# Shridhar2602/WebGPU-Path-Tracer

Measured on AMD Instinct MI355X. Metric: Mrays/s at 1080p, 8 bounces; achieved HBM GB/s vs roofline, higher is better.
Workload: dtype f32; 1 GPU; configs[1]: Cornell + monkey_968.obj (967 tris), 1920x1080, 64 spp, 8 bounces, stack_size 20; parallelism=1 GPU

## Files before the change

### webgpu-path-tracer_amd/csrc/ptmi.hip

```cpp
#include <dlfcn.h>
#include <hip/hip_runtime.h>
#include <rccl/rccl.h>

#include <algorithm>
#include <chrono>
#include <cmath>
#include <cstdio>
#include <cstdlib>
#include <condition_variable>
#include <cstring>
#include <functional>
#include <mutex>
#include <string>
#include <thread>
#include <vector>

#include "../../include/ptmi.h"
#include "ptmi_kernels.h"

using namespace ptmi;

int ptmi_bvhdev_build_scene(void* stream, const float* d_tris, uint32_t n, const int32_t* h_meshes, int n_meshes, const float* h_xforms, int n_xforms, float* d_rows,
                            float* d_tris_out, int* depth_out, uint32_t* bad_tri, int sah, uint32_t* n_nodes_out);
int ptmi_bvhdev_make_pairs(void* stream, const float* d_rows, uint32_t nn, float* d_pairs, int* d_leaf_table, uint32_t* n_multi);
// ... 49 lines not shown
  void loop() {
    std::unique_lock<std::mutex> lk(m);
    for (;;) {
      cv.wait(lk, [this] { return has_job || quit; });
      if (quit) return;
      std::function<int()> j = std::move(job);
      has_job = false;
      lk.unlock();
      const int r = j();
      lk.lock();
      result = r;
      done = true;
      cv.notify_all();
    }
  }
  void post(std::function<int()> j) {
    std::lock_guard<std::mutex> lk(m);
    if (!th.joinable()) th = std::thread([this] { loop(); });
    job = std::move(j);
    has_job = true;
    done = false;
    cv.notify_all();
  }
  int wait() {
    std::unique_lock<std::mutex> lk(m);
    cv.wait(lk, [this] { return done; });
    return result;
  }
  ~PeerWorker() {
    {
      std::lock_guard<std::mutex> lk(m);
      quit = true;
      cv.notify_all();
    }
    if (th.joinable()) th.join();
  }
};

struct Tuning {
  int lds_stack = 10;
  bool noabort = true;
  int waves_per_cu = 0;
  int bvh_teams = 16;
  int refill = kRefillThreshold, leaf_batch = kLeafBatch, bvh_range = (int)kBvhRange;
  int tail_waves_per_cu = 0;
  bool tail6 = true;
  int tail_park = 16;
  int bvh_carry = 32;
  int bvh_carry_slots = 1 << 18;
  int bvh_carry_last = 0;
  int bvh_carry_min_paths = 4 << 20, bvh_carry_min_depth = 12;
  int sort = -1;
  int shade_blocks_per_cu = 0;
  int tail_limit = -1;
  bool render_ahead = true;
  int path_budget_log2 = 30;
  int placement_tries = 6;
  bool debug_placement = false;
};

struct ptmi_ctx {
  int device = 0;
  hipStream_t stream = nullptr;
  std::string err;
  ptmi_params prm;
  Tuning tun;
  int num_cus = 256;

  std::vector<float> h_spheres, h_quads, h_xforms, h_mats, h_bvh;
  size_t n_tris_uploaded = 0;
  std::vector<int32_t> h_meshes;
  bool scene_dirty = true;

  DBuf d_quad_unit_n;
  DBuf d_bvh_rows;
  bool bvh_on_device = false;
  size_t bvh_dev_prims = 0;
  size_t bvh_dev_nodes = 0;
  bool bvh_dev_sah = false;
  bool bvh_dev_stale = false;
  int bvh_dev_depth = 0;
  DBuf d_spheres, d_sphere_info, d_quads, d_quad_mat, d_tris, d_pretri, d_trinorm, d_meshes, d_xforms, d_mats, d_pairs, d_leaf_table;
  DevScene S{};
  int bvh_depth = 0;
  bool has_unknown_material = false;
  int material_classes = 0;
  int shade_blocks_per_cu[16] = {0};

  int W = 0, H = 0;
  DBuf d_fb_own;
  float4* fb = nullptr;
  size_t fb_bytes = 0;
  int rank = 0, world = 1, tile = 64;

  size_t path_cap = 0;
  bool pixsum_alloc = false;
  size_t slot_cap = 0;
  DBuf d_q0[2], d_q1[2], d_q2[2], d_tp[2], d_hm[2];
  DBuf d_uv, d_acc, d_pixsum, d_touched, d_ctl, d_totals, d_scratch, d_spill, d_heads;
  DBuf d_carry[2];
  int ctl_cap = 0;

  struct Ahead {
    bool valid = false;
    float view[16];
    uint32_t frame0 = 0;
// ... 423 lines not shown
  const int a = step & 1, b = a ^ 1;
  P.in = Slots{c->d_q0[a].as<float4>(), c->d_q1[a].as<float4>(), c->d_q2[a].as<float4>()};
  P.out = Slots{c->d_q0[b].as<float4>(), c->d_q1[b].as<float4>(), c->d_q2[b].as<float4>()};
  P.hin = HitBuf{c->d_tp[a].as<float2>(), c->d_hm[a].as<uint32_t>()};
  P.hout = HitBuf{c->d_tp[b].as<float2>(), c->d_hm[b].as<uint32_t>()};
  P.uv = c->d_uv.as<float2>();
  P.acc = c->d_acc.as<float4>();
  P.pixsum = with_pixsum ? c->d_pixsum.as<float4>() : nullptr;
  P.touched = with_pixsum ? nullptr : c->d_touched.as<uint8_t>();
  P.cap = (uint32_t)c->slot_cap;
  return P;
}

const void* shade_kernel(bool is, bool so, bool cn, bool mu) {
  if (!is && !mu) {
    if (so) return cn ? reinterpret_cast<const void*>(&k_shade6<true, true>) : reinterpret_cast<const void*>(&k_shade6<true, false>);
    return cn ? reinterpret_cast<const void*>(&k_shade6<false, true>) : reinterpret_cast<const void*>(&k_shade6<false, false>);
  }
#define PTMI_SK(I, S, C, M) \
  if (is == I && so == S && cn == C && mu == M) return reinterpret_cast<const void*>(&k_shade<I, S, C, M>)
  PTMI_SK(false, false, false, true); PTMI_SK(false, false, true, true);
  PTMI_SK(false, true, false, true); PTMI_SK(false, true, true, true);
  PTMI_SK(true, false, false, false); PTMI_SK(true, false, false, true); PTMI_SK(true, false, true, false); PTMI_SK(true, false, true, true);
  PTMI_SK(true, true, false, false); PTMI_SK(true, true, false, true); PTMI_SK(true, true, true, false); PTMI_SK(true, true, true, true);
#undef PTMI_SK
  return nullptr;
}

int stack_alloc_for(const ptmi_ctx* c) { return std::max(1, std::min(c->prm.stack_size, std::max(c->bvh_depth, 1))); }

int env_int(const char* name, int dflt) {
  const char* v = getenv(name);
  return (v && *v) ? atoi(v) : dflt;
}
void load_tuning(ptmi_ctx* c) {
  Tuning t;
  t.lds_stack = std::max(1, env_int("PTMI_LDS_STACK", t.lds_stack));
  t.noabort = env_int("PTMI_NOABORT", 1) != 0;
  t.waves_per_cu = env_int("PTMI_WAVES_PER_CU", 0);
  t.bvh_teams = (int)std::max<uint32_t>(1, std::min<uint32_t>(kMaxTeams, (uint32_t)env_int("PTMI_BVH_TEAMS", t.bvh_teams)));
  t.refill = env_int("PTMI_REFILL", t.refill);
  t.leaf_batch = env_int("PTMI_LEAF_BATCH", t.leaf_batch);
  t.bvh_range = std::max(64, std::min(1 << 16, env_int("PTMI_BVH_RANGE", t.bvh_range))) & ~63;
  t.tail_waves_per_cu = std::max(0, std::min(32, env_int("PTMI_TAIL_WAVES_PER_CU", t.tail_waves_per_cu)));
  t.tail6 = env_int("PTMI_TAIL6", 1) != 0;
  t.tail_park = std::max(0, std::min(63, env_int("PTMI_TAIL_PARK", t.tail_park)));
  t.bvh_carry = std::max(0, env_int("PTMI_BVH_CARRY", t.bvh_carry));
  t.bvh_carry_slots = std::max(64, std::min(1 << 22, env_int("PTMI_BVH_CARRY_SLOTS", t.bvh_carry_slots)));
  t.bvh_carry_last = std::max(0, env_int("PTMI_BVH_CARRY_LAST", t.bvh_carry_last));
  t.bvh_carry_min_paths = std::max(0, env_int("PTMI_BVH_CARRY_MIN_PATHS", t.bvh_carry_min_paths));
  t.bvh_carry_min_depth = std::max(0, env_int("PTMI_BVH_CARRY_MIN_DEPTH", t.bvh_carry_min_depth));
  t.sort = env_int("PTMI_SORT", -1);
  t.shade_blocks_per_cu = env_int("PTMI_SHADE_BLOCKS_PER_CU", 0);
  t.tail_limit = env_int("PTMI_TAIL_LIMIT", -1);
  t.render_ahead = env_int("PTMI_RENDER_AHEAD", 1) != 0;
  t.path_budget_log2 = std::max(16, std::min(31, env_int("PTMI_PATH_BUDGET_LOG2", t.path_budget_log2)));
  t.placement_tries = env_int("PTMI_PLACEMENT_TRIES", t.placement_tries);
  t.debug_placement = getenv("PTMI_DEBUG_PLACEMENT") != nullptr;
  c->tun = t;
}

int launch_intersect(ptmi_ctx* c, const Paths& P, StepCtl* ctl, uint32_t max_items, bool with_prims, const RenderConst* first_rc = nullptr, const Carry& cy = Carry{}) {
  unsigned long long* tot = c->d_totals.as<unsigned long long>();
  const uint32_t pgrid = std::max<uint32_t>(1, std::min<uint32_t>((max_items + kBlock - 1) / kBlock, (uint32_t)c->num_cus * 32));
  if (with_prims) {
    ScopedSpan sp(c, T_PRIMS);
    if (c->counters) hipLaunchKernelGGL(k_prims<true>, dim3(pgrid), dim3(kBlock), 0, c->stream, c->S, P, ctl, c->d_heads.as<uint32_t>(), tot);
    else hipLaunchKernelGGL(k_prims<false>, dim3(pgrid), dim3(kBlock), 0, c->stream, c->S, P, ctl, c->d_heads.as<uint32_t>(), tot);
  }
  if (c->S.n_nodes <= 0) return PTMI_OK;
  ScopedSpan sp(c, T_BVH);
  const Tuning& tun = c->tun;
  const int sa = stack_alloc_for(c);
  const int le = std::min(sa, tun.lds_stack);
  const int se = sa - le;
  const size_t lds = (size_t)le * 2 * 64 * sizeof(int) + kCandSlots * sizeof(uint32_t);
  const bool noabort = c->bvh_depth < c->prm.stack_size && tun.noabort;
  int waves_per_cu = (int)std::min<size_t>(28, (size_t)(160 * 1024) / (lds + 64));
  if (tun.waves_per_cu > 0) waves_per_cu = tun.waves_per_cu;
  const uint32_t want = (max_items + 63) / 64;
  const uint32_t grid = std::max<uint32_t>(1, std::min<uint32_t>(want, (uint32_t)c->num_cus * (uint32_t)waves_per_cu));
  const uint32_t n_teams = (uint32_t)tun.bvh_teams;
  HIP_TRY(c, c->d_spill.ensure(std::max<size_t>(16, (size_t)std::max<uint32_t>(grid, (uint32_t)c->num_cus * 32) * (size_t)se * 64 * sizeof(int2))));
  const int thr = tun.refill, leaf_batch = tun.leaf_batch;
  const uint32_t range_cap = (uint32_t)tun.bvh_range;
  float4 cam = make_float4(0.0f, 0.0f, 0.0f, 0.0f);
  if (first_rc) cam = make_float4(first_rc->cam_o[0], first_rc->cam_o[1], first_rc->cam_o[2], 1.0f);
#define PTMI_LAUNCH_BVH(CNT, NA)                                                                                                                                       \
  hipLaunchKernelGGL((k_bvh2<CNT, NA>), dim3(grid), dim3(64), lds, c->stream, c->S, P, ctl, c->d_heads.as<uint32_t>(), n_teams, c->prm.stack_size, le, se, \
                     c->d_spill.as<int2>(), thr, leaf_batch, tot, range_cap, cam, cy)
  if (c->counters) {
    if (noabort) PTMI_LAUNCH_BVH(true, true);
    else PTMI_LAUNCH_BVH(true, false);
  } else {
    if (noabort) PTMI_LAUNCH_BVH(false, true);
    else PTMI_LAUNCH_BVH(false, false);
  }
#undef PTMI_LAUNCH_BVH
  HIP_TRY(c, hipGetLastError());
  return PTMI_OK;
}

int launch_tail(ptmi_ctx* c, const RenderConst& rc, const Paths& P, StepCtl* ctl, int first, uint32_t limit, const Carry& cy_in) {
  Carry cy = cy_in;
  cy.park_below = (c->S.n_nodes > 0 && c->bvh_depth >= 12) ? c->tun.tail_park : 0;
  const int sa = stack_alloc_for(c) + (cy.park_below > 0 ? 3 : 0);
// ... 130 lines not shown
    for (int k = 0; k < 10; k++) {
      if (ok && cand[k].p) {
        losers.bufs.emplace_back();
        std::swap(losers.bufs.back(), cand[k]);
      } else {
        cand[k].release();
      }
    }
    if (!ok) break;
  }
  restore.stats.placement_sets = sets;
  restore.stats.placement_ms = std::chrono::duration<double, std::milli>(std::chrono::steady_clock::now() - t_search).count();
  return rc_out;
}

int render_batch(ptmi_ctx* c, const float* view16, uint32_t frame0, int n_frames, int reset_first, int fold = -1, int dry_steps = 0) {
  const ptmi_params& p = c->prm;
  c->ahead.valid = false;
  RenderConst rc{};
  rc.W = (float)c->W;
  rc.H = (float)c->H;
  memcpy(rc.view, view16, 64);
  {
    const float* m = rc.view;
    for (int k = 0; k < 3; k++) rc.cam_o[k] = ((m[k] * 0.0f + m[4 + k] * 0.0f) + m[8 + k] * 0.0f) + m[12 + k] * 1.0f;
  }
  rc.fov_factor = (float)(1.0 / std::tan((double)p.fov_degrees * (3.14159265358979323846 / 180.0) / 2.0));
  rc.bg[0] = p.background[0], rc.bg[1] = p.background[1], rc.bg[2] = p.background[2];
  rc.max_bounces = p.max_bounces;
  rc.stratify = p.stratify ? 1 : 0;
  if (p.stratify) {
    float sqrt_spp = (float)std::sqrt((double)p.num_samples);
    int side = 0;
    for (float i = 0.0f; i < sqrt_spp; i += 1.0f) side++;
    rc.strat_side = side;
    rc.recip_sqrt_spp = 1.0f / (float)(int)sqrt_spp;
    rc.num_samples = side * side;
    rc.sample_div = (float)(side * side);
  } else {
    rc.strat_side = 1;
    rc.recip_sqrt_spp = 1.0f;
    rc.num_samples = p.num_samples;
    rc.sample_div = (float)p.num_samples;
  }
  rc.stack_size = p.stack_size;
  rc.light_mix = p.light_mix;
  rc.surface_mix = 1.0f - p.light_mix;
  rc.npix = (uint32_t)c->W * (uint32_t)c->H;
  rc.frame0 = frame0;
  rc.n_frames = n_frames;
  rc.reset_first = reset_first;
  rc.rank = c->rank, rc.world = c->world, rc.tile = c->tile;
  rc.n_local = count_local(rc.npix, c->rank, c->world, c->tile);
  if (rc.n_local == 0) return PTMI_OK;

  const int n_steps = rc.num_samples * p.max_bounces;
  const size_t npaths = (size_t)rc.n_local * (size_t)n_frames;
  c->batch_enqueued = false;
  int rcode = ensure_paths(c, npaths, n_steps + 2, rc.num_samples > 1);
  if (rcode) return rcode;
  StepCtl* ctl = c->d_ctl.as<StepCtl>();
  const uint32_t total = rc.n_local * (uint32_t)n_frames;
  const int sa_carry = stack_alloc_for(c);
  const bool carry = c->tun.bvh_carry > 0 && c->S.n_nodes > 0 && c->bvh_depth >= c->tun.bvh_carry_min_depth && total >= (uint32_t)c->tun.bvh_carry_min_paths && p.max_bounces > 1;
  const uint32_t resv = carry ? (uint32_t)c->tun.bvh_carry_slots : 0u;
  const int rec_words = 8 + 2 * sa_carry;
  if (carry)
    for (int k = 0; k < 2; k++) HIP_TRY(c, c->d_carry[k].ensure((size_t)resv * (size_t)rec_words * 4));
  auto carry_of = [&](int s) {
    Carry cy{};
    cy.resv = s == 0 ? 0u : resv;
    cy.resv_next = resv;
    cy.after = c->tun.bvh_carry;
    cy.rec_words = rec_words;
    cy.pool_in = c->d_carry[s & 1].as<uint32_t>();
    cy.pool_out = c->d_carry[(s + 1) & 1].as<uint32_t>();
    return cy;
  };
  const uint32_t bound = total + total / 8 + (uint32_t)c->num_cus * 8 * 1024 + resv;
  const uint32_t ew_grid = std::max<uint32_t>(1, std::min<uint32_t>((total + kBlock - 1) / kBlock, (uint32_t)c->num_cus * 16));
  const int sort_env = c->tun.sort;
  const bool sort = sort_env >= 0 ? sort_env != 0 : c->material_classes > 1;

  const bool shade_multi = rc.num_samples > 1;
  int shade_bpc = c->tun.shade_blocks_per_cu;
  if (shade_bpc <= 0) {
    int& cached = c->shade_blocks_per_cu[(p.importance_sampling ? 8 : 0) | (sort ? 4 : 0) | (c->counters ? 2 : 0) | (shade_multi ? 1 : 0)];
    if (cached == 0) {
      int nb = 0;
      if (hipOccupancyMaxActiveBlocksPerMultiprocessor(&nb, shade_kernel(p.importance_sampling != 0, sort, c->counters, shade_multi), kBlock, 0) != hipSuccess || nb < 1) nb = 5;
      cached = nb;
    }
    shade_bpc = cached;
  }
  const uint32_t sgrid = std::max<uint32_t>(1, std::min<uint32_t>((bound + kSChunk - 1) / kSChunk, (uint32_t)c->num_cus * (uint32_t)std::min(8, std::max(1, shade_bpc))));
  unsigned long long* tot = c->d_totals.as<unsigned long long>();
  const int tail_env = c->tun.tail_limit;
  const bool six = !p.importance_sampling && rc.num_samples == 1 && c->S.n_spheres == 0 && c->tun.tail6;
  const bool shallow = six && c->S.n_nodes > 0 && c->bvh_depth < 12, deep = six && c->S.n_nodes > 0 && c->bvh_depth >= 12 && c->tun.tail_park > 0;
  const uint32_t tail_limit_first = (uint32_t)(tail_env >= 0 ? tail_env : shallow ? kTailLimitFirstShallow : deep ? kTailLimitFirstDeep : kTailLimitFirst),
                 tail_limit_later = (uint32_t)(tail_env >= 0 ? tail_env : shallow ? kTailLimitLaterShallow : kTailLimitLater);

  if (dry_steps == 0 && c->placement_pending) {
    c->placement_pending = false;
    if (total > tail_limit_first) {
      int r = placement_search(c, [&]() { return render_batch(c, view16, frame0, n_frames, reset_first, fold, 2); });
// ... 1184 lines not shown
```

### webgpu-path-tracer_amd/csrc/ptmi_device.h

```cpp
#pragma once
#include <hip/hip_runtime.h>
#include <stdint.h>

#include "../../include/ptmi_math.h"

#define DEV __device__ __forceinline__

namespace ptmi {

#ifdef PTMI_LANE_TALLY
constexpr int kLaneTallies = 48;
__shared__ uint32_t s_lane_tally[kLaneTallies * 2];
__device__ unsigned long long g_lane_tally[kLaneTallies * 2];
template <int K>
DEV void lane_tally() {
  static_assert(K >= 0 && K < kLaneTallies, "tally point out of range");
  const unsigned long long m = __ballot(1);
  asm volatile("; LT_MARK %0" ::"n"(K));
  if (__builtin_amdgcn_mbcnt_hi((uint32_t)(m >> 32), __builtin_amdgcn_mbcnt_lo((uint32_t)m, 0u)) == 0u) {
    atomicAdd(&s_lane_tally[2 * K], 1u);
    atomicAdd(&s_lane_tally[2 * K + 1], (uint32_t)__popcll(m));
  }
}
#define LT(k) lane_tally<k>()
constexpr int kTimeTallies = 12;
__shared__ unsigned long long s_time_tally[4 * kTimeTallies];
__shared__ unsigned long long s_time_last[4];
__device__ unsigned long long g_time_tally[2 * kTimeTallies];
template <int K>
DEV void time_tally(float dep) {
  unsigned long long now;
  asm volatile("s_memtime %0\n\ts_waitcnt lgkmcnt(0)" : "=s"(now) : "v"(dep) : "memory");
  const unsigned long long m = __ballot(1);
  if (__builtin_amdgcn_mbcnt_hi((uint32_t)(m >> 32), __builtin_amdgcn_mbcnt_lo((uint32_t)m, 0u)) == 0u) {
    const uint32_t wv = threadIdx.x >> 6;
    const unsigned long long last = s_time_last[wv];
    if (last) atomicAdd(&s_time_tally[wv * kTimeTallies + K], now - last);
    s_time_last[wv] = now;
  }
}
#define TT(k, dep) time_tally<k>(dep)
#else
#define LT(k) ((void)0)
#define TT(k, dep) ((void)0)
#endif
enum : int { TT_OTHER = 0, TT_LOAD1 = 1, TT_LOAD2 = 2, TT_SHADE = 3, TT_STAGE = 4, TT_FLUSH_PRIMS = 5, TT_FLUSH_STORE = 6, TT_RING_READ = 7 };
enum : int {
  LT_GROUP = 0, LT_VALID = 1, LT_MISS = 2, LT_HIT = 3, LT_RH_SPHERE = 4, LT_RH_VOLUME = 5, LT_RH_QUAD = 6, LT_RH_TRI = 7, LT_MS_LAMBERT = 8, LT_MS_MIRROR = 9,
  LT_MS_GLASS = 10, LT_MS_ISO = 11, LT_RR = 12, LT_ACC_CONT = 13, LT_END_SAMPLE = 14, LT_END_CHANGES = 15, LT_FLUSH = 16, LT_QUAD_LOOP = 17, LT_QUAD_FRONT = 18,
  LT_QUAD_DENOM = 19, LT_QUAD_T = 20, LT_QUAD_ACCEPT = 21, LT_ROOT_BOX = 22, LT_MISS_SHORTCUT = 23, LT_KEEP = 24, LT_DIV3_SLOW = 25, LT_RCP_SLOW = 26, LT_SQRT_SLOW = 27,
  LT_SPHERE_LOOP = 28, LT_IS_LIGHT = 29, LT_STAGE = 30
};

constexpr float kPi = 3.14159265358979323846;
constexpr float kTwoPi = 2.0 * 3.14159265358979323846;
constexpr float kMinFloat = 0.0001;
constexpr float kMaxFloat = 999999999.999;
constexpr float kMaxFloatP1 = 999999999.999 + 1;

enum : uint32_t { K_NONE = 0, K_SPHERE = 1, K_VOLUME = 2, K_QUAD = 3, K_TRI = 4 };
enum : int { BIN_LAMBERTIAN = 0, BIN_MIRROR = 1, BIN_GLASS = 2, BIN_ISOTROPIC = 3, BIN_OTHER = 4, BIN_MISS = 5, NUM_BINS = 6 };

struct f3 {
  float x, y, z;
};
DEV f3 mk3(float x, float y, float z) { return f3{x, y, z}; }
DEV f3 mk3(float4 v) { return f3{v.x, v.y, v.z}; }
DEV f3 operator+(f3 a, f3 b) { return mk3(a.x + b.x, a.y + b.y, a.z + b.z); }
DEV f3 operator-(f3 a, f3 b) { return mk3(a.x - b.x, a.y - b.y, a.z - b.z); }
DEV f3 operator*(f3 a, f3 b) { return mk3(a.x * b.x, a.y * b.y, a.z * b.z); }
DEV f3 operator*(f3 a, float s) { return mk3(a.x * s, a.y * s, a.z * s); }
DEV f3 operator*(float s, f3 a) { return mk3(s * a.x, s * a.y, s * a.z); }
__device__ __attribute__((noinline)) f3 div3_ieee(f3 a, float s) {
  LT(LT_DIV3_SLOW);
  return mk3(a.x / s, a.y / s, a.z / s);
}
DEV f3 operator/(f3 a, float s) {
  const double ds = (double)s;
  double r = __builtin_amdgcn_rcp(ds);
  const double e = __builtin_fma(-ds, r, 1.0);
  r = __builtin_fma(r, __builtin_fma(e, e, e), r);
  f3 q = mk3((float)((double)a.x * r), (float)((double)a.y * r), (float)((double)a.z * r));
  constexpr int kDenorm = 0x090, kZeroInfNan = 0x267;
  if (__builtin_amdgcn_class(s, kZeroInfNan) | __builtin_amdgcn_class(q.x, kDenorm) | __builtin_amdgcn_class(q.y, kDenorm) | __builtin_amdgcn_class(q.z, kDenorm))
    q = div3_ieee(a, s);
  return q;
}
DEV f3 operator-(f3 a) { return mk3(-a.x, -a.y, -a.z); }

__device__ __attribute__((noinline)) float rcp_ieee_slow(float x) {
  LT(LT_RCP_SLOW);
  return 1.0f / x;
}
__device__ __attribute__((noinline)) float sqrt_ieee_slow(float x) {
  LT(LT_SQRT_SLOW);
  return __builtin_sqrtf(x);
}
DEV float rcp_core(float x) {
  const float y0 = __builtin_amdgcn_rcpf(x);
  return __builtin_fmaf(__builtin_fmaf(-x, y0, 1.0f), y0, y0);
}
DEV bool rcp_in_range(uint32_t bits) { return ((bits & 0x7fffffffu) - (27u << 23)) < (200u << 23); }
DEV float rcp_exact(float x) {
  float r = rcp_core(x);
// ... 120 lines not shown
};
struct Paths {
  Slots in, out;
  HitBuf hin, hout;
  float2* uv;
  float4* acc;
  float4* pixsum;
  uint8_t* touched;
  uint32_t cap;
};

struct alignas(128) StepCtl {
  uint32_t n_rays;
  uint32_t tail_done;
  uint32_t n_carried;
  uint32_t pad[29];
};
struct Carry {
  uint32_t resv;
  uint32_t resv_next;
  int after;
  int rec_words;
  uint32_t* pool_in;
  uint32_t* pool_out;
  int park_below;
};
DEV bool dead_slot(uint32_t slot, uint32_t n_carried, uint32_t resv) { return slot >= n_carried && slot < resv; }
constexpr int kTallyLines = 32;
constexpr size_t kTotalsBytes = 128 + (size_t)kTallyLines * 128;
DEV uint32_t* tally_line(unsigned long long* totals, uint32_t k) {
  return reinterpret_cast<uint32_t*>(totals + 16) + (k % (uint32_t)kTallyLines) * 32u;
}

struct RenderConst {
  float W, H;
  float view[16];
  float cam_o[3];
  float fov_factor;
  float bg[3];
  int max_bounces;
  int num_samples;
  int stratify;
  int strat_side;
  float recip_sqrt_spp;
  float sample_div;
  int stack_size;
  float light_mix, surface_mix;
  uint32_t npix;
  uint32_t frame0;
  int n_frames;
  int reset_first;
  uint32_t n_local;
  int rank, world, tile;
};

DEV uint32_t local_to_pixel(const RenderConst& rc, uint32_t j) {
  uint32_t tl = j / (uint32_t)rc.tile, within = j - tl * (uint32_t)rc.tile;
  return (tl * (uint32_t)rc.world + (uint32_t)rc.rank) * (uint32_t)rc.tile + within;
}

DEV f3 cam_origin(const RenderConst& rc) { return mk3(rc.cam_o[0], rc.cam_o[1], rc.cam_o[2]); }

DEV void camera_pixel(const RenderConst& rc, uint32_t pix, float& px, float& py) {
  const float W = rc.W;
  float fidx = (float)pix;
  float q = fidx / W;
  px = fidx - W * truncf(q);
  py = q;
}
DEV void camera_ray_at(const RenderConst& rc, float px, float py, int k, uint32_t& rng, f3& o, f3& d) {
  const float W = rc.W, H = rc.H;
  float a, b;
  if (rc.stratify) {
    float i = (float)(k / rc.strat_side), j = (float)(k % rc.strat_side);
    a = (W / H) * (2.0f * ((px - 0.5f + (rc.recip_sqrt_spp * (i + rand2D(rng)))) / W) - 1.0f);
    b = -1.0f * (2.0f * ((py - 0.5f + (rc.recip_sqrt_spp * (j + rand2D(rng)))) / H) - 1.0f);
  } else {
    a = (W / H) * (2.0f * ((px - 0.5f + rand2D(rng)) / W) - 1.0f);
    b = -1.0f * (2.0f * ((py - 0.5f + rand2D(rng)) / H) - 1.0f);
  }
  const float* m = rc.view;
  float nf = -rc.fov_factor;
  float dx = ((m[0] * a + m[4] * b) + m[8] * nf) + m[12] * 0.0f;
  float dy = ((m[1] * a + m[5] * b) + m[9] * nf) + m[13] * 0.0f;
  float dz = ((m[2] * a + m[6] * b) + m[10] * nf) + m[14] * 0.0f;
  float dw = ((m[3] * a + m[7] * b) + m[11] * nf) + m[15] * 0.0f;
  float len = sqrt_exact(((dx * dx + dy * dy) + dz * dz) + dw * dw);
  d = mk3(dx, dy, dz) / len;
  o = cam_origin(rc);
}
DEV void camera_ray(const RenderConst& rc, uint32_t pix, int k, uint32_t& rng, f3& o, f3& d) {
  float px, py;
  camera_pixel(rc, pix, px, py);
  camera_ray_at(rc, px, py, k, rng, o, d);
}

#define PTMI_CONST_AS __attribute__((address_space(4)))
typedef float v4f_t __attribute__((ext_vector_type(4)));
typedef int v2i_t __attribute__((ext_vector_type(2)));
DEV float4 ldu(const float4* p) {
  const v4f_t v = *(const PTMI_CONST_AS v4f_t*)(p);
  return make_float4(v.x, v.y, v.z, v.w);
}
DEV int2 ldu(const int2* p) {
  const v2i_t v = *(const PTMI_CONST_AS v2i_t*)(p);
  return make_int2(v.x, v.y);
// ... 491 lines not shown
```

### webgpu-path-tracer_amd/csrc/ptmi_kernels.h

```cpp
#pragma once
#include "ptmi_device.h"

namespace ptmi {

constexpr int kBlock = 256;

constexpr uint32_t kHeadStride = 32, kMaxTeams = 64;
DEV void reset_heads(uint32_t* __restrict__ heads) {
  if (blockIdx.x == 0 && threadIdx.x < kMaxTeams) heads[threadIdx.x * kHeadStride] = 0u;
}

DEV void reduce_counters(const Counters& cn, unsigned long long* __restrict__ totals, bool bvh) {
  uint32_t v[5] = {cn.node_visits, cn.tri_tests, cn.sphere_tests, cn.quad_tests, cn.mat_fetches};
#pragma unroll
  for (int k = 0; k < 5; k++) {
    unsigned long long x = v[k];
    for (int off2 = 32; off2 > 0; off2 >>= 1) x += __shfl_down(x, off2, 64);
    if (lane_id() == 0 && x) {
      atomicAdd(&totals[2 + k], x);
      if (bvh && k == 0) atomicAdd(&totals[7], x);
      if (bvh && k == 4) atomicAdd(&totals[8], x);
    }
  }
}
// ... 447 lines not shown
          T = T * rcp_exact(p);
        }
      }
      if (!sample_done) {
        bounce++;
        if (bounce >= rc.max_bounces) sample_done = true;
      }
    }
  }

  const bool changes = !(add.x == 0.0f && add.y == 0.0f && add.z == 0.0f);
  ns.pid = pid;
  if (!sample_done) {
    if (changes) {
      LT(LT_ACC_CONT);
      float4 A4 = acc_load(P, pid, acc_written);
      f3 acc = mk3(A4) + add;
      acc_store(P, pid, make_float4(acc.x, acc.y, acc.z, A4.w), acc_written);
      acc_written = true;
    }
    ns.o = no, ns.d = nd, ns.T = T, ns.bounce = bounce | (acc_written ? kAccWritten : 0), ns.rng = rng;
    return true;
  }

  LT(LT_END_SAMPLE);
  if (!MULTI) {
    if (drop_acc) {
      f3 fin = mk3(0, 0, 0) + add;
      acc_store(P, pid, make_float4(fin.x, fin.y, fin.z, __int_as_float(1)), acc_written);
    } else {
      end_sample_progressive(P, pid, add, acc_written);
    }
    return false;
  } else {
  float4 A4 = P.acc[pid];
  int sample = __float_as_int(A4.w);
  f3 radiance = drop_acc ? add : (mk3(A4) + add);
  f3 sum = mk3(P.pixsum[pid]) + radiance;
  sample++;
  if (sample < rc.num_samples) {
    P.pixsum[pid] = make_float4(sum.x, sum.y, sum.z, 0.0f);
    camera_ray(rc, local_to_pixel(rc, pid % rc.n_local), sample, rng, no, nd);
    P.acc[pid] = make_float4(0.0f, 0.0f, 0.0f, __int_as_float(sample));
    ns.o = no, ns.d = nd, ns.T = mk3(1.0f, 1.0f, 1.0f), ns.bounce = 0, ns.rng = rng;
    return true;
  }
  f3 fin = sum / rc.sample_div;
  P.acc[pid] = make_float4(fin.x, fin.y, fin.z, __int_as_float(sample));
  return false;
  }
}

constexpr uint32_t kRegionDiv = 16;
constexpr int kTailLimitFirst = 2 << 20, kTailLimitLater = 1 << 20;
constexpr int kTailLimitFirstShallow = 24 << 20, kTailLimitLaterShallow = 2 << 20;
constexpr int kTailLimitFirstDeep = 6 << 20;
constexpr int kTailRefill = 16;
constexpr bool kMissShortcut = true;
constexpr int kSChunk = 512;

template <bool IS, bool COUNT, bool MULTI>
DEV void shade_body(const DevScene& S, const RenderConst& rc, const Paths& P, StepCtl* __restrict__ ctl, uint32_t* __restrict__ heads, unsigned long long* __restrict__ totals,
                    int first, uint32_t resv) {
  reset_heads(heads);
  __shared__ float4 s_q0[kSChunk], s_q1[kSChunk], s_q2[kSChunk];
  __shared__ uint16_t s_sorted[kSChunk];
  __shared__ uint32_t s_cnt[NUM_BINS + 2];
  __shared__ uint32_t s_nout, s_next;
  const QuadL L = load_light(S);
  const int lane = lane_id();
  const uint32_t n_carried = resv ? min(ctl->n_carried, resv) : 0u;
  uint32_t n = ctl->n_rays;
  if (n <= resv && n_carried == 0u) n = 0u;
  const uint32_t region = max((uint32_t)kSChunk, ((n / gridDim.x / kRegionDiv) + 511u) & ~511u);
  const uint32_t wregion = region / (kBlock / 64);
  uint32_t w_cur = 0, w_rend = 0;
  constexpr uint32_t kR0Empty = 0xffffffffu, kR0Busy = 0xfffffffeu, kR0Full = 0xfffffffdu;
  __shared__ uint32_t s_region0;
  if (threadIdx.x == 0) s_region0 = kR0Empty;
  uint32_t my_valid = 0;
  uint32_t my_missed = 0;
  Counters cn = {0, 0, 0, 0, 0};
  auto stage = [&](bool survive, const NewState& ns) {
    const uint64_t mk = __ballot(survive);
    if (mk) {
      const int leader = __ffsll((unsigned long long)mk) - 1;
      uint32_t bb = 0;
      if (lane == leader) bb = atomicAdd(&s_nout, (uint32_t)__popcll(mk));
      bb = (uint32_t)__shfl((int)bb, leader, 64);
      if (survive) {
        const uint32_t q = bb + lanes_below(mk);
        s_q0[q] = make_float4(ns.o.x, ns.o.y, ns.o.z, __uint_as_float(ns.rng));
        s_q1[q] = make_float4(ns.d.x, ns.d.y, ns.d.z, __uint_as_float(ns.pid));
        s_q2[q] = make_float4(ns.T.x, ns.T.y, ns.T.z, __int_as_float(ns.bounce));
      }
    }
  };
  for (uint32_t base = blockIdx.x * (uint32_t)kSChunk; base < n; base += gridDim.x * (uint32_t)kSChunk) {
    const uint32_t m = min((uint32_t)kSChunk, n - base);
    if (threadIdx.x < NUM_BINS) s_cnt[threadIdx.x] = 0;
    if (threadIdx.x == 0) {
      s_nout = 0;
      s_next = 0;
    }
    __syncthreads();
    {
// ... 126 lines not shown
      }
      if (keep && (rank < n0 || b1 != 0xffffffffu)) {
        const uint32_t dst = (rank < n0) ? (b0 + rank) : (b1 + (rank - n0));
        float4 a0 = s_q0[q];
        a0.w = __uint_as_float(rng);
        P.out.q0[dst] = a0;
        P.out.q1[dst] = s_q1[q];
        P.out.q2[dst] = s_q2[q];
        P.hout.tp[dst] = tp;
        P.hout.mat[dst] = hm;
      }
    }
    if (!MULTI) {
      for (int off2 = 32; off2 > 0; off2 >>= 1) missed += __shfl_down(missed, off2, 64);
      if (lane == 0) my_missed += missed;
    }
    __syncthreads();
  }
  if (lane == 0 && my_missed + my_valid) atomicAdd(tally_line(totals, blockIdx.x), my_missed + my_valid);
  if (w_rend == 0u && blockIdx.x * (uint32_t)kSChunk < n && s_region0 < kR0Full) {
    w_cur = s_region0 + (threadIdx.x >> 6) * wregion;
    w_rend = w_cur + wregion;
  }
  for (uint32_t i = w_cur + (uint32_t)lane; i < w_rend; i += 64u) {
    reinterpret_cast<uint32_t*>(P.out.q1 + i)[3] = PID_HOLE;
    P.hout.mat[i] = HITMAT_HOLE;
  }
  if (COUNT) reduce_counters(cn, totals, false);
}

template <bool IS, bool COUNT, bool MULTI>
DEV void shade_body_wave(const DevScene& S, const RenderConst& rc, const Paths& P, StepCtl* __restrict__ ctl, uint32_t* __restrict__ heads,
                         unsigned long long* __restrict__ totals, int first, uint32_t resv) {
  reset_heads(heads);
  constexpr uint32_t kRing = 128, kWaves = kBlock / 64;
  static_assert((size_t)kWaves * kRing == (size_t)kSChunk, "the rings take the LDS the block version's staging arrays take");
  __shared__ float4 s_q0[kWaves * kRing], s_q1[kWaves * kRing], s_q2[kWaves * kRing];
  constexpr uint32_t kR0Empty = 0xffffffffu, kR0Busy = 0xfffffffeu, kR0Full = 0xfffffffdu;
  __shared__ uint32_t s_region0;
  if (threadIdx.x == 0) s_region0 = kR0Empty;
#ifdef PTMI_LANE_TALLY
  if (threadIdx.x < kLaneTallies * 2) s_lane_tally[threadIdx.x] = 0u;
  if (threadIdx.x < 4 * kTimeTallies) s_time_tally[threadIdx.x] = 0ull;
  if (threadIdx.x < 4) s_time_last[threadIdx.x] = 0ull;
#endif
  __syncthreads();
  const QuadL L = load_light(S);
  const int lane = lane_id();
  const uint32_t wv = threadIdx.x >> 6;
  float4 *const r0 = s_q0 + wv * kRing, *const r1 = s_q1 + wv * kRing, *const r2 = s_q2 + wv * kRing;
  const uint32_t n_carried = resv ? min(ctl->n_carried, resv) : 0u;
  uint32_t n = ctl->n_rays;
  if (n <= resv && n_carried == 0u) n = 0u;
  const uint32_t region = max((uint32_t)kSChunk, ((n / gridDim.x / kRegionDiv) + 511u) & ~511u);
  const uint32_t wregion = region / kWaves;
  uint32_t w_cur = 0, w_rend = 0;
  uint32_t head = 0, cnt = 0;
  uint32_t my_valid = 0, my_missed = 0;
  Counters cn = {0, 0, 0, 0, 0};
  auto flush_pass = [&](uint32_t take) {
    const uint32_t q = (head + (uint32_t)lane) & (kRing - 1u);
    bool keep = false;
    float2 tp = make_float2(0.0f, 0.0f);
    uint32_t hm = 0u, rng = 0u;
    if ((uint32_t)lane < take) {
      LT(LT_FLUSH);
      const float4 a0 = r0[q], a1 = r1[q];
      TT(TT_RING_READ, a0.x + a1.x);
      rng = __float_as_uint(a0.w);
      prims_for_ray<COUNT>(S, mk3(a0), mk3(a1), rng, tp, hm, cn);
      TT(TT_FLUSH_PRIMS, tp.x + __uint_as_float(hm));
      if (kMissShortcut && !MULTI && hm == HITMAT_MISS) {
        LT(LT_MISS_SHORTCUT);
        const float4 a2 = r2[q];
        end_sample_progressive(P, __float_as_uint(a1.w), mk3(rc.bg[0], rc.bg[1], rc.bg[2]) * mk3(a2), (__float_as_int(a2.w) & kAccWritten) != 0);
      } else {
        keep = true;
      }
    }
    const uint64_t km = __ballot(keep);
    const uint32_t kept = (uint32_t)__popcll(km);
    my_missed += take - kept;
    if (kept) {
      const uint32_t rank = lanes_below(km);
      const uint32_t b0 = w_cur, n0 = min(kept, w_rend - w_cur);
      uint32_t b1 = 0xffffffffu;
      w_cur += n0;
      if (kept > n0) {
        uint32_t nb = 0;
        bool full;
        if (w_rend == 0u) {
          if (lane == 0) nb = atomicCAS(&s_region0, kR0Empty, kR0Busy);
          nb = (uint32_t)__builtin_amdgcn_readfirstlane((int)nb);
          if (nb == kR0Empty) {
            if (lane == 0) {
              nb = atomicAdd(&ctl[1].n_rays, region);
              if (nb + region > P.cap) {
                atomicAdd(&totals[15], 1ull);
                atomicSub(&ctl[1].n_rays, region);
                nb = kR0Full;
              }
              atomicExch(&s_region0, nb);
            }
            nb = (uint32_t)__builtin_amdgcn_readfirstlane((int)nb);
          } else {
            while (nb == kR0Busy) {
              __builtin_amdgcn_s_sleep(8);
              if (lane == 0) nb = atomicAdd(&s_region0, 0u);
              nb = (uint32_t)__builtin_amdgcn_readfirstlane((int)nb);
            }
          }
          full = nb == kR0Full;
          nb += wv * wregion;
        } else {
          if (lane == 0) nb = atomicAdd(&ctl[1].n_rays, wregion);
          nb = (uint32_t)__builtin_amdgcn_readfirstlane((int)nb);
          full = nb + wregion > P.cap;
          if (full && lane == 0) {
            atomicAdd(&totals[15], 1ull);
            atomicSub(&ctl[1].n_rays, wregion);
          }
        }
        if (!full) {
          b1 = nb;
          w_cur = nb + (kept - n0);
          w_rend = nb + wregion;
        }
      }
      if (keep && (rank < n0 || b1 != 0xffffffffu)) {
        LT(LT_KEEP);
        const uint32_t dst = (rank < n0) ? (b0 + rank) : (b1 + (rank - n0));
        float4 a0 = r0[q];
        a0.w = __uint_as_float(rng);
        P.out.q0[dst] = a0;
        P.out.q1[dst] = r1[q];
        P.out.q2[dst] = r2[q];
        P.hout.tp[dst] = tp;
        P.hout.mat[dst] = hm;
      }
    }
    head = (head + take) & (kRing - 1u);
    cnt -= take;
    TT(TT_FLUSH_STORE, 0.0f);
  };
  auto shade_group = [&](bool active, const SlotState& st) {
    bool survive = false, valid = false;
    NewState ns;
    ns.o = ns.d = ns.T = mk3(0, 0, 0);
    ns.bounce = 0, ns.rng = 0, ns.pid = 0;
    TT(TT_OTHER, 0.0f);
    if (active) {
      LT(LT_GROUP);
      TT(TT_LOAD1, st.q0.x + st.q1.x + st.q2.x + st.tp.x + __uint_as_float(st.hitmat));
      valid = __float_as_uint(st.q1.w) != PID_HOLE;
      if (valid) {
        LT(LT_VALID);
        const TriFetch tf = tri_fetch(S, P.uv, st.slot, __float_as_uint(st.tp.y));
        survive = shade_one<IS, MULTI>(S, rc, P, st, tf, L, ns);
      }
    }
    TT(TT_SHADE, ns.o.x + ns.T.x);
    my_valid += (uint32_t)__popcll(__ballot(valid));
    const uint64_t mk = __ballot(survive);
    if (survive) {
      LT(LT_STAGE);
      const uint32_t q = (head + cnt + lanes_below(mk)) & (kRing - 1u);
      r0[q] = make_float4(ns.o.x, ns.o.y, ns.o.z, __uint_as_float(ns.rng));
      r1[q] = make_float4(ns.d.x, ns.d.y, ns.d.z, __uint_as_float(ns.pid));
      r2[q] = make_float4(ns.T.x, ns.T.y, ns.T.z, __int_as_float(ns.bounce));
    }
    cnt += (uint32_t)__popcll(mk);
    TT(TT_STAGE, 0.0f);
  };
  {
    uint32_t base = blockIdx.x * (uint32_t)kSChunk, j0 = wv * 64u;
    auto settle = [&]() {
      while (base < n && j0 >= min((uint32_t)kSChunk, n - base)) {
        base += gridDim.x * (uint32_t)kSChunk;
        j0 = wv * 64u;
      }
      return base < n;
    };
    auto fetch = [&](SlotState& st) {
      const uint32_t j = j0 + (uint32_t)lane;
      const bool act = j < min((uint32_t)kSChunk, n - base) && !dead_slot(base + j, n_carried, resv);
      if (act) st = load_slot(P, base + j, first != 0, rc);
      return act;
    };
    SlotState cur;
    bool have = settle(), cur_act = false;
    if (have) cur_act = fetch(cur);
#pragma unroll 1
    while (have) {
      shade_group(cur_act, cur);
      j0 += kBlock;
      have = settle();
      SlotState nxt;
      bool nxt_act = false;
      if (have) nxt_act = fetch(nxt);
      if (cnt >= 64u) flush_pass(64u);
      cur = nxt;
      cur_act = nxt_act;
    }
  }
  if (cnt) flush_pass(cnt);
  if (MULTI) my_missed = 0;
  if (lane == 0 && my_missed + my_valid) atomicAdd(tally_line(totals, blockIdx.x), my_missed + my_valid);
  __syncthreads();
#ifdef PTMI_LANE_TALLY
  if (threadIdx.x < kLaneTallies * 2 && s_lane_tally[threadIdx.x]) atomicAdd(&g_lane_tally[threadIdx.x], (unsigned long long)s_lane_tally[threadIdx.x]);
  if (threadIdx.x < kTimeTallies) {
    unsigned long long t = 0;
    for (int w = 0; w < 4; w++) t += s_time_tally[w * kTimeTallies + threadIdx.x];
    if (t) atomicAdd(&g_time_tally[threadIdx.x], t);
  }
#endif
  if (w_rend == 0u && s_region0 < kR0Full) {
    w_cur = s_region0 + wv * wregion;
    w_rend = w_cur + wregion;
  }
  for (uint32_t i = w_cur + (uint32_t)lane; i < w_rend; i += 64u) {
    reinterpret_cast<uint32_t*>(P.out.q1 + i)[3] = PID_HOLE;
    P.hout.mat[i] = HITMAT_HOLE;
  }
  if (COUNT) reduce_counters(cn, totals, false);
}

template <bool IS, bool SORT, bool COUNT, bool MULTI>
__global__ __launch_bounds__(kBlock) PTMI_SHADE_ATTR void k_shade(DevScene S, RenderConst rc, Paths P, StepCtl* __restrict__ ctl, uint32_t* __restrict__ heads,
                                                                  unsigned long long* __restrict__ totals, int first, uint32_t resv) {
  if constexpr (SORT) shade_body<IS, COUNT, MULTI>(S, rc, P, ctl, heads, totals, first, resv);
  else shade_body_wave<IS, COUNT, MULTI>(S, rc, P, ctl, heads, totals, first, resv);
}
template <bool SORT, bool COUNT>
__global__ __launch_bounds__(kBlock) __attribute__((amdgpu_waves_per_eu(6, 8))) void k_shade6(DevScene S, RenderConst rc, Paths P, StepCtl* __restrict__ ctl,
                                                                                                uint32_t* __restrict__ heads, unsigned long long* __restrict__ totals, int first, uint32_t resv) {
  if constexpr (SORT) shade_body<false, COUNT, false>(S, rc, P, ctl, heads, totals, first, resv);
  else shade_body_wave<false, COUNT, false>(S, rc, P, ctl, heads, totals, first, resv);
}

constexpr int kTailTravBatch = 24;
template <bool IS, bool COUNT, bool MULTI, bool NOABORT>
DEV void tail_body(const DevScene& S, const RenderConst& rc, const Paths& P, StepCtl* __restrict__ ctl, unsigned long long* __restrict__ totals, int first, uint32_t limit,
                   int stack_size, int lds_entries, int spill_entries, int2* __restrict__ spill, const Carry& cy) {
  const uint32_t n_carried = cy.resv ? min(ctl->n_carried, cy.resv) : 0u;
  const uint32_t n = ctl->n_rays;
  if (n <= cy.resv && n_carried == 0u) return;
  if ((n > cy.resv ? n - cy.resv : 0u) + n_carried > limit) return;
  extern __shared__ int lds_stack[];
  const int lane = lane_id();
  LaneStack2 stk;
  stk.lds = (lds_v2i_t*)lds_stack + lane;
  stk.spill = spill + (size_t)blockIdx.x * (size_t)spill_entries * 64 + lane;
  stk.lds_entries = lds_entries;
  const QuadL L = load_light(S);
  Counters cn = {0, 0, 0, 0, 0}, cb = {0, 0, 0, 0, 0};
  uint32_t tally = 0;
  const uint32_t root = __float_as_uint(S.root_lo.w);
  const uint32_t root_node = (root & REF_LEAF) ? root : (root & REF_IDX);
  SlotState st;
  st.q0 = st.q1 = st.q2 = make_float4(0.0f, 0.0f, 0.0f, 0.0f);
  st.tp = make_float2(0.0f, 0.0f);
  st.hitmat = HITMAT_HOLE, st.slot = 0;
  bool alive = false;
  bool resume = false;
  int park_sp = -1;
  float2 uv = make_float2(0.0f, 0.0f);
  uint32_t gnext = blockIdx.x, gbase = 0, pos = 64;
#ifdef PTMI_LANE_TALLY
  unsigned long long bt_cyc[kBvhTallies] = {0}, bt_last;
  uint32_t bt_marks[kBvhTallies] = {0}, bt_lanes[kBvhTallies] = {0};
  asm volatile("s_memtime %0\n\ts_waitcnt lgkmcnt(0)" : "=s"(bt_last)::"memory");
#endif
#pragma unroll 1
  for (;;) {
    BT(TB_VOTE, 0.0f, 0);
    uint64_t am = __ballot(alive);
// ... 365 lines not shown
```

Baseline: 26400 Mrays/s.

## Continue shading fully resolved hits in-wave instead of writing them back

In the wave-based shade kernel, when at least shade_cont lanes of a flush group hold final (non-BVH) hits, those rays are shaded again right away in the same wave rather than written to the output ring for the next step. Output regions are also allocated in smaller chunks when continuation is enabled, which reduces hole padding. The aim is to save global stores, reloads and extra step iterations for rays that need no further traversal. The cost is extra ballots and control divergence, register pressure from the carried state, and a different ordering of work.

```diff
diff --git a/webgpu-path-tracer_amd/csrc/ptmi.hip b/webgpu-path-tracer_amd/csrc/ptmi.hip
--- a/webgpu-path-tracer_amd/csrc/ptmi.hip
+++ b/webgpu-path-tracer_amd/csrc/ptmi.hip
@@ -125,6 +125,7 @@
   int bvh_carry_min_paths = 4 << 20, bvh_carry_min_depth = 12;
   int sort = -1;
   int shade_blocks_per_cu = 0;
+  int shade_cont = 16;
   int tail_limit = -1;
   bool render_ahead = true;
   int path_budget_log2 = 30;
@@ -654,6 +655,7 @@
   t.bvh_carry_min_depth = std::max(0, env_int("PTMI_BVH_CARRY_MIN_DEPTH", t.bvh_carry_min_depth));
   t.sort = env_int("PTMI_SORT", -1);
   t.shade_blocks_per_cu = env_int("PTMI_SHADE_BLOCKS_PER_CU", 0);
+  t.shade_cont = std::max(0, std::min(64, env_int("PTMI_SHADE_CONT", t.shade_cont)));
   t.tail_limit = env_int("PTMI_TAIL_LIMIT", -1);
   t.render_ahead = env_int("PTMI_RENDER_AHEAD", 1) != 0;
   t.path_budget_log2 = std::max(16, std::min(31, env_int("PTMI_PATH_BUDGET_LOG2", t.path_budget_log2)));
@@ -890,6 +892,7 @@
   rc.reset_first = reset_first;
   rc.rank = c->rank, rc.world = c->world, rc.tile = c->tile;
   rc.n_local = count_local(rc.npix, c->rank, c->world, c->tile);
+  rc.shade_cont = (uint32_t)c->tun.shade_cont;
   if (rc.n_local == 0) return PTMI_OK;
 
   const int n_steps = rc.num_samples * p.max_bounces;
diff --git a/webgpu-path-tracer_amd/csrc/ptmi_device.h b/webgpu-path-tracer_amd/csrc/ptmi_device.h
--- a/webgpu-path-tracer_amd/csrc/ptmi_device.h
+++ b/webgpu-path-tracer_amd/csrc/ptmi_device.h
@@ -49,7 +49,7 @@
   LT_GROUP = 0, LT_VALID = 1, LT_MISS = 2, LT_HIT = 3, LT_RH_SPHERE = 4, LT_RH_VOLUME = 5, LT_RH_QUAD = 6, LT_RH_TRI = 7, LT_MS_LAMBERT = 8, LT_MS_MIRROR = 9,
   LT_MS_GLASS = 10, LT_MS_ISO = 11, LT_RR = 12, LT_ACC_CONT = 13, LT_END_SAMPLE = 14, LT_END_CHANGES = 15, LT_FLUSH = 16, LT_QUAD_LOOP = 17, LT_QUAD_FRONT = 18,
   LT_QUAD_DENOM = 19, LT_QUAD_T = 20, LT_QUAD_ACCEPT = 21, LT_ROOT_BOX = 22, LT_MISS_SHORTCUT = 23, LT_KEEP = 24, LT_DIV3_SLOW = 25, LT_RCP_SLOW = 26, LT_SQRT_SLOW = 27,
-  LT_SPHERE_LOOP = 28, LT_IS_LIGHT = 29, LT_STAGE = 30
+  LT_SPHERE_LOOP = 28, LT_IS_LIGHT = 29, LT_STAGE = 30, LT_CONT = 31, LT_HOLE = 32
 };
 
 constexpr float kPi = 3.14159265358979323846;
@@ -276,6 +276,7 @@
   int reset_first;
   uint32_t n_local;
   int rank, world, tile;
+  uint32_t shade_cont;
 };
 
 DEV uint32_t local_to_pixel(const RenderConst& rc, uint32_t j) {
diff --git a/webgpu-path-tracer_amd/csrc/ptmi_kernels.h b/webgpu-path-tracer_amd/csrc/ptmi_kernels.h
--- a/webgpu-path-tracer_amd/csrc/ptmi_kernels.h
+++ b/webgpu-path-tracer_amd/csrc/ptmi_kernels.h
@@ -523,6 +523,7 @@
 }
 
 constexpr uint32_t kRegionDiv = 16;
+constexpr uint32_t kRegionDivCont = 64;
 constexpr int kTailLimitFirst = 2 << 20, kTailLimitLater = 1 << 20;
 constexpr int kTailLimitFirstShallow = 24 << 20, kTailLimitLaterShallow = 2 << 20;
 constexpr int kTailLimitFirstDeep = 6 << 20;
@@ -755,13 +756,16 @@
   const uint32_t n_carried = resv ? min(ctl->n_carried, resv) : 0u;
   uint32_t n = ctl->n_rays;
   if (n <= resv && n_carried == 0u) n = 0u;
-  const uint32_t region = max((uint32_t)kSChunk, ((n / gridDim.x / kRegionDiv) + 511u) & ~511u);
-  const uint32_t wregion = region / kWaves;
+  const uint32_t cont_min = MULTI ? 0u : rc.shade_cont;
+  const uint32_t region_full = max((uint32_t)kSChunk, ((n / gridDim.x / kRegionDiv) + 511u) & ~511u);
+  const uint32_t region = cont_min ? max((uint32_t)kSChunk, ((n / gridDim.x / kRegionDivCont) + 511u) & ~511u) : region_full;
+  const uint32_t wregion = region / kWaves, wregion_full = region_full / kWaves;
+  bool pred = true;
   uint32_t w_cur = 0, w_rend = 0;
   uint32_t head = 0, cnt = 0;
   uint32_t my_valid = 0, my_missed = 0;
   Counters cn = {0, 0, 0, 0, 0};
-  auto flush_pass = [&](uint32_t take) {
+  auto flush_pass = [&](uint32_t take, SlotState& cs, bool cont) {
     const uint32_t q = (head + (uint32_t)lane) & (kRing - 1u);
     bool keep = false;
     float2 tp = make_float2(0.0f, 0.0f);
@@ -781,16 +785,25 @@
         keep = true;
       }
     }
+    bool go = false;
+    if (cont_min) {
+      const bool final_hit = keep && (hm & HITMAT_BVH) == 0u;
+      pred = (uint32_t)__popcll(__ballot(final_hit)) >= cont_min;
+      if (cont && pred) {
+        go = final_hit;
+        keep = keep && !final_hit;
+      }
+    }
     const uint64_t km = __ballot(keep);
     const uint32_t kept = (uint32_t)__popcll(km);
-    my_missed += take - kept;
+    my_missed += take - kept - (uint32_t)__popcll(__ballot(go));
     if (kept) {
       const uint32_t rank = lanes_below(km);
       const uint32_t b0 = w_cur, n0 = min(kept, w_rend - w_cur);
       uint32_t b1 = 0xffffffffu;
       w_cur += n0;
       if (kept > n0) {
-        uint32_t nb = 0;
+        uint32_t nb = 0, wregion_next = wregion;
         bool full;
         if (w_rend == 0u) {
           if (lane == 0) nb = atomicCAS(&s_region0, kR0Empty, kR0Busy);
@@ -816,18 +829,20 @@
           full = nb == kR0Full;
           nb += wv * wregion;
         } else {
-          if (lane == 0) nb = atomicAdd(&ctl[1].n_rays, wregion);
+          const uint32_t wr = pred ? wregion : wregion_full;
+          if (lane == 0) nb = atomicAdd(&ctl[1].n_rays, wr);
           nb = (uint32_t)__builtin_amdgcn_readfirstlane((int)nb);
-          full = nb + wregion > P.cap;
+          full = nb + wr > P.cap;
           if (full && lane == 0) {
             atomicAdd(&totals[15], 1ull);
-            atomicSub(&ctl[1].n_rays, wregion);
+            atomicSub(&ctl[1].n_rays, wr);
           }
+          wregion_next = wr;
         }
         if (!full) {
           b1 = nb;
           w_cur = nb + (kept - n0);
-          w_rend = nb + wregion;
+          w_rend = nb + wregion_next;
         }
       }
       if (keep && (rank < n0 || b1 != 0xffffffffu)) {
@@ -842,9 +857,20 @@
         P.hout.mat[dst] = hm;
       }
     }
+    if (cont) {
+      if (go) LT(LT_CONT);
+      cs.q0 = r0[q];
+      cs.q0.w = __uint_as_float(rng);
+      cs.q1 = r1[q];
+      cs.q2 = r2[q];
+      cs.tp = tp;
+      cs.hitmat = hm;
+      cs.slot = 0u;
+    }
     head = (head + take) & (kRing - 1u);
     cnt -= take;
     TT(TT_FLUSH_STORE, 0.0f);
+    return go;
   };
   auto shade_group = [&](bool active, const SlotState& st) {
     bool survive = false, valid = false;
@@ -891,22 +917,30 @@
       return act;
     };
     SlotState cur;
-    bool have = settle(), cur_act = false;
+    bool have = settle(), cur_act = false, again = false;
     if (have) cur_act = fetch(cur);
 #pragma unroll 1
-    while (have) {
+    while (have || again) {
       shade_group(cur_act, cur);
-      j0 += kBlock;
-      have = settle();
+      if (!again) {
+        j0 += kBlock;
+        have = settle();
+      }
+      const bool flush_due = cnt >= 64u;
+      const bool pre = have && !(cont_min && flush_due && pred);
       SlotState nxt;
       bool nxt_act = false;
-      if (have) nxt_act = fetch(nxt);
-      if (cnt >= 64u) flush_pass(64u);
+      if (pre) nxt_act = fetch(nxt);
+      bool go = false;
+      if (flush_due) go = flush_pass(64u, nxt, cont_min != 0u && !pre);
+      again = __ballot(go) != 0ull;
+      if (again) nxt_act = go;
+      else if (have && !pre) nxt_act = fetch(nxt);
       cur = nxt;
       cur_act = nxt_act;
     }
-  }
-  if (cnt) flush_pass(cnt);
+    if (cnt) flush_pass(cnt, cur, false);
+  }
   if (MULTI) my_missed = 0;
   if (lane == 0 && my_missed + my_valid) atomicAdd(tally_line(totals, blockIdx.x), my_missed + my_valid);
   __syncthreads();
@@ -923,9 +957,14 @@
     w_rend = w_cur + wregion;
   }
   for (uint32_t i = w_cur + (uint32_t)lane; i < w_rend; i += 64u) {
+    LT(LT_HOLE);
     reinterpret_cast<uint32_t*>(P.out.q1 + i)[3] = PID_HOLE;
     P.hout.mat[i] = HITMAT_HOLE;
   }
+#ifdef PTMI_LANE_TALLY
+  __syncthreads();
+  if (threadIdx.x >= 2 * LT_HOLE && threadIdx.x < 2 * LT_HOLE + 2 && s_lane_tally[threadIdx.x]) atomicAdd(&g_lane_tally[threadIdx.x], (unsigned long long)s_lane_tally[threadIdx.x]);
+#endif
   if (COUNT) reduce_counters(cn, totals, false);
 }
 
```

Result: faster. 29150 Mrays/s (median of 6 runs) (+10.4%).
